# viswavi/speech-anonymization

Hardware: AMD Instinct MI355X
Metric: audio frames/sec (node), ConvAE+gender-adv train step (higher is better)
Workload: dtype bf16x3; 1 GPU; ConvAE recon0.1+sex0.9 adversarial train step (L1 recon + NLL), shape M: 32 utt/GPU x 161120 samples (T=1008 frames), Fbank x2 + norm + fwd + bwd + clip + Adam + Noam; batch_per_gpu=32, frames_per_utt=1008, parallelism=dp1

## Files before the change

include/sa_hip.h:

```cpp
#ifndef SA_HIP_H
#define SA_HIP_H
#ifdef __cplusplus
extern "C" {
#endif

#define SA_F32 0
#define SA_BF16 1
#define SA_BF16X3 2
#define SA_BF16X1F 3
#define SA_FP8 4
#define SA_F64 5
#define SA_MAX_TAPS 5
#define SA_COMM_ID_BYTES 128

typedef struct SaTaps {
  int ntaps[2];
  int off[2][SA_MAX_TAPS];
  int widx[2][SA_MAX_TAPS];
} SaTaps;

typedef struct SaConvArgs {
  const void* x;
  const void* wp;
  const float* bias;
// ... 27 lines not shown
int sa_conv_gemm_route(int dtype, int cin, int cout, int sa, int u, const SaConvArgs* a);

int sa_pack_weights(int dtype, const float* src, void* dst, int ntaps, int K, int N, int sk, int sn,
                    int st, void* stream);

typedef struct SaPackDesc {
  const float* src; void* dst;
  int dtype, ntaps, K, N, sk, sn, st, pad_;
  float* scale;
} SaPackDesc;
int sa_pack_weights_multi(const SaPackDesc* descs, int n, int blocks_per_image, void* stream);
int sa_pack_scales_multi(const SaPackDesc* descs, int n, void* stream);

typedef struct SaWgradArgs {
  const void* x;
  const void* dy;
  float* slabs;
  const float* s1; const float* t1; const float* s2; const float* t2; int swish;
  int B, Lin, Ldy, Mrows, chunk, nchunk;
  int ntaps; int off[SA_MAX_TAPS]; int ph[SA_MAX_TAPS];
  int x_pre;
  int dy_pre;
} SaWgradArgs;

int sa_wgrad(int dtype, int cin, int cout, int sa, int u, const SaWgradArgs* a, void* stream);
int sa_wgrad_kw(int cin, int cout);
int sa_wgrad_reduce(const float* slabs, float* dst, int nslab, int ntaps, int cin, int cout, int sk,
                    int sn, int st, int accumulate, void* stream);
#define SA_WRED_MAX 8
typedef struct SaWredDesc {
  const float* slabs; float* dst;
  int nslab, ntaps, cin, cout, sk, sn, st, accumulate, vec, pad_;
} SaWredDesc;
typedef struct SaWredMulti { int n, pad_; SaWredDesc d[SA_WRED_MAX]; } SaWredMulti;
int sa_wgrad_reduce_multi(const SaWredMulti* m, void* stream);

int sa_conv1toC(int dtype, const float* x, const float* w, const float* bias, void* y, int B, int L,
                int flip, float* stats, const void* ep_x, const float* ep_s1, const float* ep_t1,
                const float* ep_mean, const float* ep_rstd, void* stream);
int sa_conv1toC_ntiles(int L);
int sa_convCto1(int dtype, const void* x, const float* w, const float* bias, float* y, int B, int L,
                const float* s1, const float* t1, int swish, int flip, void* stream);
int sa_wgrad1C(int dtype, const float* u, const void* v, float* slabs, int B, int L, int chunk,
               int flip, const float* s1, const float* t1, int swish, void* stream);
int sa_wgrad1C_nchunk(int L, int chunk);
int sa_bwd1C(int dtype, const float* u, const void* v, const float* w, void* g, float* stats, float* slabs,
             int B, int L, int chunk, int flip, const float* s1, const float* t1, const float* mean,
             const float* rstd, void* stream);
int sa_sum_slabs(const float* slabs, float* dst, int nslab, int n, int accumulate, void* stream);

typedef struct SaEwArgs {
  const void* g; const void* g2; const void* x; void* out;
  const float* s1; const float* t1;
  const float* mean; const float* rstd;
  const float* c1; const float* c2; const float* c3;
  int actbwd, xp_is_act, relu_mask, bstride;
  float* stats;
  int B, L, ntiles;
} SaEwArgs;

int sa_ew_stats(int dtype, int C, const SaEwArgs* a, void* stream);
int sa_ew_apply(int dtype, int C, const SaEwArgs* a, void* stream);
int sa_ew_ntiles(int L);
int sa_sum_partials(const float* slabs, double* dst, int nbatch, int nslab, int n, void* stream);
int sa_sum_rows_d(const double* src, double* dst, int R, int n, void* stream);
int sa_fin_in_fwd(const double* sums, int B, int C, int n, const float* gamma, const float* beta,
                  float eps, float* mean, float* rstd, float* scale, float* shift, void* stream);
int sa_fin_bn_fwd(const double* sums, int R, int C, double count, const float* gamma, const float* beta,
                  float eps, float momentum, float* run_mean, float* run_var, float* mean,
                  float* rstd, float* scale, float* shift, const double* count_dev, void* stream);
int sa_fin_bn_eval(int C, const float* gamma, const float* beta, float eps, const float* run_mean,
                   const float* run_var, float* mean, float* rstd, float* scale, float* shift,
                   void* stream);
int sa_fin_norm_bwd(const double* sums, const double* lsums, int R, int groups, int C, double n,
                    const float* gamma, const float* mean, const float* rstd, float sign, float* c1,
                    float* c2, float* c3, float* dgamma, float* dbeta, const double* n_dev,
                    void* stream);
int sa_fin_bias(const double* sums, int B, int C, int ncomp, float* db, void* stream);

#define SA_FLATS_MAX 4
typedef struct SaFlat { float* p; long long n; } SaFlat;
typedef struct SaFlats { int n, pad_; SaFlat f[SA_FLATS_MAX]; } SaFlats;
int sa_clip_grads(const SaFlats* f, float max_norm, float eps, double* partials, float* total_norm, void* stream);
#define SA_BIAS_MAX 8
typedef struct SaBiasDesc {
  const float* part; double* rows; float* db;
  int nbatch, nslab, C, ncomp;
} SaBiasDesc;
typedef struct SaBiasMulti { int n, pad_; SaBiasDesc d[SA_BIAS_MAX]; } SaBiasMulti;
int sa_bias_multi(const SaBiasMulti* m, void* stream);

int sa_pool_fwd(int dtype, const void* r, const float* scale, const float* shift, float* part, int B,
                int L, int nseg, void* stream);
int sa_pool_nseg(int B);
int sa_pool_gather(const float* part, int B, int nseg, int L, double* sums, void* stream);
int sa_pool_fin(const double* sums, int B, int n, const float* noise, float eps, float* pooled,
                float* mean, float* stdraw, void* stream);
int sa_pool_gather_fin(const float* part, int B, int nseg, int L, const float* noise, int raw, float eps,
                       float* pooled, float* mean, float* stdraw, void* stream);
int sa_pool_bwd(int dtype, const void* r, const float* scale, const float* shift,
                const float* dpooled, const float* mean, const float* stdraw, void* g, int B, int L,
                const float* bn_mean, const float* bn_rstd, float* stats, void* stream);
int sa_dense(const float* X, int lda, const float* ps, const float* pt, const float* W, int sbk,
             int sbn, const float* bias, float* Y, int ldy, int M, int N, int K, int relu,
             void* stream);
int sa_colsums(const float* X, const float* H, const float* hmean, const float* hrstd, int M, int N,
               double* sums, float* out0, float* out1, void* stream);
int sa_bn2d_bwd(const float* G, const float* H, const double* sums, double count, const float* gamma,
                const float* mean, const float* rstd, int relu_mask, int M, int N, float* dH,
                const double* count_dev, void* stream);
int sa_dense_wgrad(const float* dY, const float* X, const float* ps, const float* pt, int M, int N,
                   int K, float* dW, void* stream);
int sa_log_softmax(const float* X, float* Y, int M, int N, void* stream);
int sa_log_softmax_bwd(const float* dY, const float* Y, float* dX, int M, int N, void* stream);
int sa_loss_workspace_bytes(void);
int sa_recon_loss(const float* a, const float* b, long long n, int kind, float* grad, float* loss,
                  void* workspace, void* stream);
int sa_cls_losses(const float* logp, const long long* label, int B, int NC, float* out, float* dnll,
                  float* dconf, void* stream);
int sa_cosine_loss(const float* x1, const float* x2, int B, int S, int D, float* rowloss,
                   float* loss, float* dx1, void* stream);
int sa_recon_loss_part(const float* a, const float* b, long long n, int kind, float* grad, float gscale,
                       void* workspace, void* stream);
int sa_step_loss(const void* workspace, long long n, const float* logp, const long long* label, int B, int NC,
                 float w_recon, float w_sex, float* out, float* dlogp, int* nonfinite, void* stream);

int sa_head_fwd(const float* pooled, const float* w1, const float* b1, const float* g1, const float* be1,
                float* rm1, float* rv1, const float* w2, const float* b2, const float* g2, const float* be2,
                float* rm2, float* rv2, const float* w3, const float* b3, float* h1, float* f1, float* h2,
                float* f2, float* logp, int M, float eps, float momentum, void* stream);
int sa_head_bwd(const float* dlogp, const float* logp, const float* pooled, const float* h1, const float* f1,
                const float* h2, const float* f2, const float* w1, const float* g1, const float* w2,
                const float* g2, const float* w3, float* dw1, float* db1, float* dg1, float* dbe1, float* dw2,
                float* db2, float* dg2, float* dbe2, float* dw3, float* db3, float* dpooled, int M, void* stream);
int sa_head_bwd_wide(const float* dlogp, const float* logp, const float* pooled, const float* h1, const float* f1,
                     const float* h2, const float* f2, const float* w1, const float* g1, const float* w2,
                     const float* g2, const float* w3, float* dw1, float* db1, float* dg1, float* dbe1, float* dw2,
                     float* db2, float* dg2, float* dbe2, float* dw3, float* db3, float* dpooled, int M,
                     void* stream);
int sa_head_max_rows(void);

int sa_tdnn_fwd(const float* x, const void* wp, const float* bias, const float* bn_s, const float* bn_t,
                float* y, int B, int T, int Cin, int Cout, int Npad, int K, int dil, float slope,
                unsigned char* mask, void* stream);
int sa_time_pool(const float* x, const float* lens, const float* noise, int B, int T, int C, float eps,
                 float* out, void* stream);
int sa_leaky_affine(const float* x, const float* s, const float* t, float slope, int M, int C, float* y,
                    void* stream);
int sa_tdnn_bwd_input(const float* dy, const unsigned char* mask, const float* bn_s, const void* wp,
                      float* dxe, int B, int T, int Cy, int Cred, int Cin, int Npad, int K, int dil,
                      float slope, void* stream);
int sa_tdnn_fold(const float* dxe, float* dx, int B, int T, int C, int pad, void* stream);
int sa_time_pool_bwd(const float* x, const float* lens, const float* g, const float* pooled, int B,
                     int T, int C, float eps, float* dx, void* stream);
int sa_leaky_affine_bwd(const float* dy, const float* x, const float* s, float slope, int M, int C,
                        float* dx, void* stream);

int sa_xv_tdnn_fwd_train(const float* x, const float* s_in, const float* t_in, const void* wp, const float* bias,
                         float* z, float* part, int B, int T, int Cin, int Cout, int Npad, int K, int dil,
                         float slope, void* stream);
int sa_xv_tdnn_ntiles(int T);
int sa_xv_colsums(const float* G, const float* H, const float* hmean, const float* hrstd, const float* c1,
                  const float* c2, const float* c3, float slope, float* out, int M, int N, int rows_per,
                  double* part, void* stream);
int sa_xv_tdnn_wgrad(const float* dpre, const float* x, const float* s_in, const float* t_in, float* part, int B,
                     int T, int Cin, int Cout, int K, int dil, int nsplit, int rows_per, void* stream);
// ... 176 lines not shown
```

speech-anonymization_amd/_lib.py:

```python
import ctypes as C
import os

import torch

_HERE = os.path.dirname(os.path.abspath(__file__))
LIB_PATH = os.environ.get("SA_HIP_LIB") or os.path.join(_HERE, "libsa_hip.so")

F32, BF16, BF16X3, BF16X1F, FP8, F64 = 0, 1, 2, 3, 4, 5
MAX_TAPS = 5

c_fp = C.POINTER(C.c_float)
vp = C.c_void_p


class SaTaps(C.Structure):
    _fields_ = [("ntaps", C.c_int * 2), ("off", (C.c_int * MAX_TAPS) * 2),
                ("widx", (C.c_int * MAX_TAPS) * 2)]


class SaConvArgs(C.Structure):
    _fields_ = [("x", vp), ("wp", vp), ("bias", vp), ("y", vp),
                ("s1", vp), ("t1", vp), ("s2", vp), ("t2", vp),
                ("swish", C.c_int), ("relu", C.c_int), ("stats", vp),
                ("B", C.c_int), ("Lin", C.c_int), ("Lout", C.c_int), ("ntiles", C.c_int),
                ("rowmin", C.c_int), ("nrows", C.c_int), ("wlo_off", C.c_int), ("taps", SaTaps),
                ("ep_mode", C.c_int), ("ep_xp_is_act", C.c_int), ("ep_bstride", C.c_int),
                ("ep_x", vp), ("ep_g2", vp), ("ep_s1", vp), ("ep_t1", vp), ("ep_mean", vp), ("ep_rstd", vp),
                ("a_out", vp),
                ("nb_x", vp), ("nb_c1", vp), ("nb_c2", vp), ("nb_c3", vp),
                ("nb_bstride", C.c_int), ("nb_relu_mask", C.c_int), ("nb_colsum", vp),
                ("ep_g2k1", vp), ("ep_g2k2", vp), ("ep_g2k3", vp), ("pro_stats", vp), ("wscale", vp),
                ("tile_rows", C.c_int), ("pad2_", C.c_int)]


class SaPackDesc(C.Structure):
    _fields_ = [("src", vp), ("dst", vp), ("dtype", C.c_int), ("ntaps", C.c_int), ("K", C.c_int),
                ("N", C.c_int), ("sk", C.c_int), ("sn", C.c_int), ("st", C.c_int), ("pad_", C.c_int),
                ("scale", vp)]


class SaWgradArgs(C.Structure):
    _fields_ = [("x", vp), ("dy", vp), ("slabs", vp),
                ("s1", vp), ("t1", vp), ("s2", vp), ("t2", vp), ("swish", C.c_int),
                ("B", C.c_int), ("Lin", C.c_int), ("Ldy", C.c_int), ("Mrows", C.c_int),
                ("chunk", C.c_int), ("nchunk", C.c_int),
                ("ntaps", C.c_int), ("off", C.c_int * MAX_TAPS), ("ph", C.c_int * MAX_TAPS),
                ("x_pre", C.c_int), ("dy_pre", C.c_int)]


class SaEwArgs(C.Structure):
    _fields_ = [("g", vp), ("g2", vp), ("x", vp), ("out", vp),
                ("s1", vp), ("t1", vp), ("mean", vp), ("rstd", vp),
                ("c1", vp), ("c2", vp), ("c3", vp),
                ("actbwd", C.c_int), ("xp_is_act", C.c_int), ("relu_mask", C.c_int),
                ("bstride", C.c_int), ("stats", vp),
                ("B", C.c_int), ("L", C.c_int), ("ntiles", C.c_int)]


BIAS_MAX = 8


class SaBiasDesc(C.Structure):
    _fields_ = [("part", vp), ("rows", vp), ("db", vp),
                ("nbatch", C.c_int), ("nslab", C.c_int), ("C", C.c_int), ("ncomp", C.c_int)]


class SaBiasMulti(C.Structure):
    _fields_ = [("n", C.c_int), ("pad_", C.c_int), ("d", SaBiasDesc * BIAS_MAX)]


WRED_MAX = 8
FLATS_MAX = 4


class SaFlat(C.Structure):
    _fields_ = [("p", vp), ("n", C.c_longlong)]


class SaFlats(C.Structure):
    _fields_ = [("n", C.c_int), ("pad_", C.c_int), ("f", SaFlat * FLATS_MAX)]



class SaWredDesc(C.Structure):
    _fields_ = [("slabs", vp), ("dst", vp)] + [(k, C.c_int) for k in ("nslab", "ntaps", "cin", "cout", "sk", "sn", "st",
                                                                      "accumulate", "vec", "pad_")]


class SaWredMulti(C.Structure):
    _fields_ = [("n", C.c_int), ("pad_", C.c_int), ("d", SaWredDesc * WRED_MAX)]


SYMBOLS = [
    "sa_conv_gemm", "sa_abi_sizeof", "sa_conv_gemm_ntiles", "sa_conv_gemm_ntiles_tm", "sa_conv_gemm_set_tile_rows",
    "sa_conv_gemm_set_impl", "sa_conv_gemm_route", "sa_pack_weights", "sa_pack_weights_multi", "sa_pack_scales_multi", "sa_wgrad", "sa_wgrad_kw", "sa_wgrad_reduce",
    "sa_conv1toC", "sa_conv1toC_ntiles", "sa_convCto1", "sa_wgrad1C", "sa_wgrad1C_nchunk", "sa_bwd1C",
    "sa_sum_slabs", "sa_ew_stats", "sa_ew_apply", "sa_ew_ntiles",
    "sa_sum_partials", "sa_sum_rows_d", "sa_fin_in_fwd", "sa_fin_bn_fwd", "sa_fin_bn_eval", "sa_fin_norm_bwd", "sa_fin_bias",
    "sa_pool_fwd", "sa_pool_nseg", "sa_pool_gather", "sa_pool_fin", "sa_pool_gather_fin", "sa_pool_bwd", "sa_dense", "sa_colsums",
    "sa_bn2d_bwd", "sa_dense_wgrad", "sa_log_softmax", "sa_log_softmax_bwd",
    "sa_loss_workspace_bytes", "sa_recon_loss", "sa_cls_losses", "sa_cosine_loss", "sa_recon_loss_part", "sa_step_loss",
    "sa_tdnn_fwd", "sa_time_pool", "sa_leaky_affine", "sa_tdnn_bwd_input", "sa_tdnn_fold", "sa_time_pool_bwd",
    "sa_leaky_affine_bwd", "sa_cluster_mi", "sa_fbank", "sa_fbank_table_elems", "sa_fbank_ntiles", "sa_fbank_scratch_bytes", "sa_fbank_normalize", "sa_fbank_normalize_pair",
    "sa_comm_unique_id", "sa_comm_init", "sa_comm_world", "sa_comm_allreduce", "sa_comm_allreduce_inline", "sa_comm_join", "sa_comm_ncalls",
    "sa_comm_destroy", "sa_head_fwd", "sa_head_bwd", "sa_head_bwd_wide", "sa_head_max_rows",
    "sa_add_layernorm_fwd", "sa_layernorm_bwd", "sa_reflect_pad_fwd", "sa_reflect_pad_bwd", "sa_ln_leaky_fwd", "sa_ln_leaky_bwd", "sa_bias_multi", "sa_asr_block0_fwd", "sa_asr_block0_bwd", "sa_wgrad_reduce_multi", "sa_clip_grads",
    "sa_xv_tdnn_fwd_train", "sa_xv_tdnn_ntiles", "sa_xv_colsums", "sa_xv_tdnn_wgrad", "sa_xv_wgrad_reduce",
    "sa_xv_tdnn_dgrad", "sa_xv_pool_affine", "sa_xv_pool_affine_bwd",
    "sa_fc_tiles", "sa_fc_groups", "sa_fc_nparam", "sa_fc_nhead", "sa_fc_max_rows", "sa_fc_enc_fwd", "sa_fc_bn_fin",
    "sa_fc_mid_fwd", "sa_fc_head_fwd", "sa_fc_head_bwd", "sa_fc_mid_bwd", "sa_fc_bn_bwd_fin", "sa_fc_enc_bwd",
    "sa_fc_wreduce", "sa_fc_recon_fwd",
    "sa_wav_augment_tile", "sa_wav_augment_max_chunks", "sa_wav_abs_sums", "sa_noise_scales", "sa_wav_augment",
    "sa_specaug_warp_sums", "sa_specaug_finalize", "sa_specaug_fill",
    "sa_gl_tile", "sa_mel_to_mag", "sa_gl_istft", "sa_gl_project",
    "sa_yin_dim", "sa_yin_f0", "sa_pitch_ratio", "sa_pitch_stretch_mag", "sa_pitch_resample",
    "sa_env_dim", "sa_env_warp",
    "sa_mcadams_dim", "sa_mcadams",
    "sa_stoi_dim", "sa_stoi",
    "sa_pv_dim", "sa_pv_synth",
    "sa_contour_dim", "sa_pitch_contour", "sa_pv_synth_map", "sa_env_warp_frames", "sa_pitch_resample_map",
    "sa_f0v_dim", "sa_f0_candidates", "sa_f0_viterbi",
    "sa_f0cmp_dim", "sa_f0_compare",
    "sa_mcd_dim", "sa_mcd",
    "sa_psola_dim", "sa_psola_marks", "sa_psola_plan", "sa_psola_ola",
    "sa_formant_dim", "sa_formant_tracks", "sa_formant_compare",
    "sa_pole_warp_dim", "sa_pole_warp", "sa_formant_centre",
]

_lib = None


class SaHipError(RuntimeError):
    pass


def load():
    global _lib
    if _lib is None:
        if not os.path.exists(LIB_PATH):
            raise SaHipError(
                f"{LIB_PATH} not found: build it with `python -c 'import __graft_entry__ as g; "
                "g.build()'` (hipcc --offload-arch=gfx950). There is no CPU fallback.")
        _lib = C.CDLL(LIB_PATH)
        for s in SYMBOLS:
            getattr(_lib, s).restype = C.c_int
        _lib.sa_pv_workspace_bytes.restype = C.c_longlong
        _lib.sa_psola_workspace_bytes.restype = C.c_longlong
        for i, rec in enumerate((SaConvArgs, SaWgradArgs, SaEwArgs, SaPackDesc, SaTaps, SaBiasMulti, SaWredMulti, SaFlats)):
            if _lib.sa_abi_sizeof(i) != C.sizeof(rec):
                raise SaHipError(f"{rec.__name__}: binding has {C.sizeof(rec)} bytes, {LIB_PATH} "
                                 f"{_lib.sa_abi_sizeof(i)} -- rebuild the library (stale build?)")
    return _lib


def stream():
    return C.c_void_p(torch._C._cuda_getCurrentRawStream(torch._C._cuda_getDevice()))


def ptr(t):
    if t is None:
        return None
    assert t.is_cuda and t.is_contiguous(), "HIP kernels take contiguous device tensors"
    return C.c_void_p(t.data_ptr())


def check(rc, what):
    if rc != 0:
        raise SaHipError(f"{what} failed with code {rc}")


def dt_code(dtype):
    if dtype == torch.float32:
        return F32
    if dtype == torch.bfloat16:
        return BF16
    raise SaHipError(f"unsupported activation dtype {dtype}")


_taps_cache = {}


def make_taps(phases):
    key = tuple(tuple(p) for p in phases)
    t = _taps_cache.get(key)
    if t is not None:
        return t
    t = _taps_cache[key] = SaTaps()
    for ph, lst in enumerate(phases):
        t.ntaps[ph] = len(lst)
        for i, (off, wi) in enumerate(lst):
            t.off[ph][i] = off
            t.widx[ph][i] = wi
    return t
```

speech-anonymization_amd/brain.py:

```python
import enum
import os
import types

import torch

from . import distributed as sdist


class Stage(enum.Enum):
    TRAIN = 1
    VALID = 2
    TEST = 3


class EpochCounter:

    def __init__(self, limit):
        self.current, self.limit = 0, int(limit)

    def __iter__(self):
        return self

    def __next__(self):
        if self.current < self.limit:
            self.current += 1
            return self.current
        raise StopIteration


class NoamScheduler:

    def __init__(self, lr_initial, n_warmup_steps, model_size=None):
        self.lr_initial, self.n_warmup_steps = lr_initial, n_warmup_steps
        self.current_lr, self.n_steps = lr_initial, 0
        self.normalize = n_warmup_steps ** 0.5 if model_size is None else model_size ** (-0.5)

    def __call__(self, opt):
        self.n_steps += 1
        current_lr = getattr(opt, "_sa_host_lr", None)
        if current_lr is None:
            current_lr = opt.param_groups[0]["lr"]
        lr = self.lr_initial * self.normalize * min(self.n_steps ** (-0.5),
                                                    self.n_steps * self.n_warmup_steps ** (-1.5))
        for g in opt.param_groups:
            if torch.is_tensor(g["lr"]):
                g["lr"].fill_(lr)
            else:
                g["lr"] = lr
        opt._sa_host_lr = lr
        self.current_lr = current_lr
        return current_lr, lr

    def state_dict(self):
        return {"losses": [], "n_steps": self.n_steps}

    def load_state_dict(self, sd):
        self.n_steps = sd["n_steps"]


class Batch:

    def __init__(self, wavs, lens, gender, tokens_bos=None, ids=None):
        self.sig = (wavs, lens)
        self.gender = gender
        self.tokens_bos = (tokens_bos if tokens_bos is not None
                           else torch.ones(wavs.shape[0], 1, dtype=torch.long), lens)
        self.id = ids

    def to(self, device):
        w, l = self.sig
        tb, tl = self.tokens_bos
        out = Batch.__new__(Batch)
        out.sig = (w.to(device, non_blocking=True), l.to(device, non_blocking=True))
        out.gender = self.gender.to(device, non_blocking=True)
        out.tokens_bos = (tb.to(device, non_blocking=True), tl.to(device, non_blocking=True))
        out.id = self.id
        return out


def settle_python_heap():
    import gc
    gc.collect()
    gc.freeze()


class Brain:
    GC_FREEZE_STEP = 8

    def __init__(self, modules=None, opt_class=None, hparams=None, run_opts=None, checkpointer=None):
        run_opts = dict(run_opts or {})
        self.device = torch.device(run_opts.get("device", "cuda:0" if torch.cuda.is_available() else "cpu"))
        if self.device.type == "cuda":
            torch.cuda.set_device(self.device)
        self.max_grad_norm = float(run_opts.get("max_grad_norm", 5.0))
        self.nonfinite_patience = int(run_opts.get("nonfinite_patience", 3))
        self.lazy_finite_check = bool(run_opts.get("lazy_finite_check", True))
        self.hip_graph = bool(run_opts.get("hip_graph", False)) and self.device.type == "cuda"
        self.gc_freeze = bool(run_opts.get("gc_freeze", True))
        self.fused_clip = bool(run_opts.get("fused_clip", os.environ.get("SA_FUSED_CLIP", "1") == "1"))
        self.front_end_once = bool(run_opts.get("front_end_once", os.environ.get("SA_FRONT_END_ONCE", "1") == "1"))
        self.step_tail = bool(run_opts.get("step_tail", os.environ.get("SA_STEP_TAIL", "1") == "1"))
        self.distributed_launch = bool(run_opts.get("distributed_launch", sdist.is_distributed()))
        self.modules = torch.nn.ModuleDict(modules or {})
        self.dp_batch_sizes = run_opts.get("dp_batch_sizes", "equal")
        self.opt_class = opt_class
        self.hparams = types.SimpleNamespace(**(hparams or {}))
        self.checkpointer = checkpointer
        self.step, self.nonfinite_count, self.optimizer = 0, 0, None
        self.avg_train_loss = 0.0

    def compute_forward(self, batch, stage):
        raise NotImplementedError

    def compute_objectives(self, predictions, batch, stage):
        raise NotImplementedError

    def on_stage_start(self, stage, epoch=None):
        pass

    def on_stage_end(self, stage, stage_loss, epoch=None):
        pass

    def on_fit_start(self):
        self.modules.to(self.device)
        for m in self.modules.values():
            if hasattr(m, "dp_batch_sizes"):
                m.dp_batch_sizes = self.dp_batch_sizes
        self.init_optimizers()
        if self.checkpointer is not None:
            if self.optimizer is not None:
                self.checkpointer.add_recoverable("optimizer", self.optimizer)
            self.resumed_from = self.checkpointer.recover_if_possible(device=self.device, brain=self)

    def init_optimizers(self):
        if self.opt_class is not None and self.optimizer is None:
            params = list(self.modules.parameters())
            base = getattr(self.opt_class, "func", self.opt_class)
            given = getattr(self.opt_class, "keywords", None) or {}
            if base is torch.optim.Adam and "fused" not in given and params and all(p.is_cuda for p in params):
                try:
                    if self.hip_graph:
                        self.optimizer = self.opt_class(params, fused=True, capturable=True)
                        for g in self.optimizer.param_groups:
                            self.optimizer._sa_host_lr = float(g["lr"])
                            g["lr"] = torch.tensor(float(g["lr"]), dtype=torch.float32, device=self.device)
                    else:
                        self.optimizer = self.opt_class(params, fused=True)
                    return
                except (TypeError, RuntimeError):
                    self.hip_graph = False
            self.optimizer = self.opt_class(params)

    def check_gradients(self, loss):
        bad = self._count_nonfinite(loss)
        if bad:
            self.nonfinite_count += bad
            if self.nonfinite_count > self.nonfinite_patience:
                raise ValueError("Loss is not finite and patience is exhausted.")
            if not (self.lazy_finite_check and loss.is_cuda):
                return False
        params = getattr(self, "_clip_params", None)
        if params is None:
            params = self._clip_params = list(self.modules.parameters())
        flats = self._grad_flats(params) if self.fused_clip else None
        if flats:
            from . import ops
            ops.clip_flats(flats, self.max_grad_norm)
        else:
            torch.nn.utils.clip_grad_norm_(params, self.max_grad_norm)
        return True

    def _grad_flats(self, params):
        model = self.modules["ConvAE"] if "ConvAE" in self.modules else None
        flats = getattr(model, "_last_flats", None) if model is not None else None
        if not flats:
            return None
        spans = [(f.data_ptr(), f.data_ptr() + 4 * f.numel(), f.numel()) for f in flats]
        seen = [0] * len(flats)
        for p in params:
            g = p.grad
            if g is None:
                continue
            if g.dtype != torch.float32 or not g.is_contiguous():
                return None
            a = g.data_ptr()
            for i, (lo, hi, _) in enumerate(spans):
                if lo <= a < hi:
                    seen[i] += g.numel()
                    break
            else:
                return None
        if any(n != span[2] for n, span in zip(seen, spans)):
            return None
        return flats

    def _count_nonfinite(self, loss):
        if not (self.lazy_finite_check and loss.is_cuda):
            return 0 if bool(torch.isfinite(loss)) else 1
        st = self._finite_counter(loss.device)
        new = self._poll_nonfinite()
        if st.pop("counted", None) is not loss:
            st["dev"].add_((~torch.isfinite(loss.detach())).to(torch.int32))
        st["host"].copy_(st["dev"], non_blocking=True)
        if not torch.cuda.is_current_stream_capturing():
            st["event"].record()
            st["pending"] = True
        return new

    def _finite_counter(self, device):
        st = getattr(self, "_finite_state", None)
        if st is None:
            st = self._finite_state = dict(dev=torch.zeros((), dtype=torch.int32, device=device),
                                           host=torch.zeros((), dtype=torch.int32).pin_memory(),
                                           event=torch.cuda.Event(), seen=0, pending=False)
        return st

    def _poll_nonfinite(self, wait=False):
        st = getattr(self, "_finite_state", None)
        if st is None or not st["pending"]:
            return 0
        if wait:
            st["event"].synchronize()
        elif not st["event"].query():
            return 0
        st["pending"] = False
        total = int(st["host"])
        new, st["seen"] = total - st["seen"], total
        return max(new, 0)

    def fit_batch(self, batch):
        outputs = self.compute_forward(batch, Stage.TRAIN)
        loss = self.compute_objectives(outputs, batch, Stage.TRAIN)
        loss.backward()
        if self.check_gradients(loss):
            self.optimizer.step()
        self.optimizer.zero_grad()
        return loss.detach()

    def evaluate_batch(self, batch, stage):
        out = self.compute_forward(batch, stage=stage)
        return self.compute_objectives(out, batch, stage=stage).detach()

    def update_average(self, loss, avg_loss):
        if not loss.is_cuda:
            if torch.isfinite(loss):
                avg_loss -= avg_loss / self.step
                avg_loss += float(loss) / self.step
            return avg_loss
        if not torch.is_tensor(avg_loss):
            avg_loss = torch.full((), float(avg_loss), device=loss.device, dtype=torch.float32)
        new = avg_loss + (loss.detach().float() - avg_loss) / self.step
        return torch.where(torch.isfinite(loss), new, avg_loss)

    def fit(self, epoch_counter, train_set, valid_set=None, progressbar=False, **_):
        self.on_fit_start()
        for epoch in epoch_counter:
            self.on_stage_start(Stage.TRAIN, epoch)
            self.modules.train()
            self.nonfinite_count = 0
            self.avg_train_loss = 0.0
            self.step = 0
            for batch in train_set:
                self.step += 1
                loss = self.fit_batch(batch)
                self.avg_train_loss = self.update_average(loss, self.avg_train_loss)
                if self.gc_freeze and self.step == self.GC_FREEZE_STEP and not self.__dict__.get("_gc_frozen"):
                    settle_python_heap()
                    self._gc_frozen = True
            self.nonfinite_count += self._poll_nonfinite(wait=True)
            if self.nonfinite_count > self.nonfinite_patience:
                raise ValueError("Loss is not finite and patience is exhausted.")
            self.avg_train_loss = float(self.avg_train_loss)
            self.on_stage_end(Stage.TRAIN, self.avg_train_loss, epoch)
            if valid_set is not None:
                self.on_stage_start(Stage.VALID, epoch)
                self.modules.eval()
                avg, n = 0.0, 0
                with torch.no_grad():
                    for batch in valid_set:
                        n += 1
                        avg += (float(self.evaluate_batch(batch, Stage.VALID)) - avg) / n
                self.on_stage_end(Stage.VALID, avg, epoch)

    def on_evaluate_start(self, max_key=None, min_key=None):
        pass

    def evaluate(self, test_set, max_key=None, min_key=None, **_):
        self.on_evaluate_start(max_key=max_key, min_key=min_key)
        self.on_stage_start(Stage.TEST, None)
        self.modules.eval()
        avg, n = 0.0, 0
        with torch.no_grad():
            for batch in test_set:
                n += 1
                avg += (float(self.evaluate_batch(batch, Stage.TEST)) - avg) / n
        self.on_stage_end(Stage.TEST, avg, None)
        return avg


class SexAnonymizationTraining(Brain):

    @staticmethod
    def _sig_key(wavs, wav_lens):
        return tuple((t.data_ptr(), tuple(t.shape), t.dtype, t._version) for t in (wavs, wav_lens))

    def features(self, wavs, wav_lens):
        stash, self._target_stash = self.__dict__.get("_target_stash"), None
        if stash is not None and stash[0] == self._sig_key(wavs, wav_lens):
            return stash[1]
        feats = self.hparams.compute_features(wavs)
        current_epoch = self.hparams.epoch_counter.current
        pad = 36 if self.hparams.model_type != "fcae" else None
        return self.modules.normalize(feats, wav_lens, epoch=current_epoch, pad_multiple=pad)

    def _features_pair(self, wavs, wav_lens):
        feats = self.hparams.compute_features(wavs)
        pad = 36 if self.hparams.model_type != "fcae" else None
        inp, target = self.modules.normalize.forward_pair(feats, wav_lens, epoch=self.hparams.epoch_counter.current,
# ... 86 lines not shown
                and isinstance(hp.loss_sex_classification, losses.NLLLoss)):
            return False
        w = (hp.recon_loss_weight, hp.sex_loss_weight, hp.utility_loss_weight)
        if not all(isinstance(x, (int, float)) and x == x and abs(x) != float("inf") for x in w):
            return False
        if not (w[2] == 0 or (w[2] > 0 and getattr(self, "asr_brain", None) is None)):
            return False
        if predictions is not None:
            recon, logp = predictions
            return bool(recon.is_cuda and recon.requires_grad and logp.requires_grad and logp.dim() == 2
                        and recon.dtype == logp.dtype == torch.float32)
        return True

    def _objectives_native(self, recon, logp, feats, label):
        from . import ops
        hp = self.hparams
        B = recon.shape[0]
        st = self._finite_counter(recon.device) if self.lazy_finite_check else None
        label = torch.as_tensor(label, device=logp.device).long().contiguous()
        out, d_recon, d_logp = ops.step_loss(
            recon.detach().view(B, -1).contiguous(), feats.detach().view(B, -1).contiguous().float(),
            hp.loss_reconstruction.kind, logp.detach().contiguous(), label,
            float(hp.recon_loss_weight), float(hp.sex_loss_weight), nonfinite=st["dev"] if st else None)
        loss = out[2]
        self.last_losses = dict(recon=out[0], sex=out[1])
        self._tail = (loss, (recon, logp), (d_recon.view_as(recon), d_logp))
        if st is not None:
            st["counted"] = loss
        return loss

    def _backward(self, loss, accumulate=False):
        tail, self._tail = self.__dict__.get("_tail"), None
        if tail is not None and tail[0] is loss:
            torch.autograd.backward(tail[1], tail[2])
        elif accumulate:
            (loss / self.hparams.gradient_accumulation).backward()
        else:
            loss.backward()

    def apply_epoch_schedule(self):
        hp = self.hparams
        if not getattr(hp, "epoch_parity_schedule", False):
            return
        joint = hp.epoch_counter.current % 2 == 0
        if joint:
            hp.recon_loss_weight, hp.sex_loss_weight = 0.0, 0.8
            hp.utility_loss_weight, hp.confusion_loss_weight = 0.2, 0.0
        else:
            hp.recon_loss_weight, hp.sex_loss_weight, hp.utility_loss_weight = 0.0, 0.5, 0.0
        for name, param in self.modules.ConvAE.named_parameters():
            param.requires_grad = ("sex_classifier" not in name) if joint else ("sex_classifier" in name)

    def _zero_grads_of_frozen(self):
        st = self.optimizer.state
        for group in self.optimizer.param_groups:
            for p in group["params"]:
                if p.grad is None and not p.requires_grad and p in st and len(st[p]):
                    z = getattr(self, "_zero_grad_cache", None)
                    if z is None:
                        z = self._zero_grad_cache = {}
                    g = z.get(p)
                    if g is None:
                        g = z[p] = torch.zeros_like(p)
                    p.grad = g

    GRAPH_WARMUP = 3

    def _graph_key(self, batch):
        hp = self.hparams
        wavs, lens = batch.sig
        nrm = self.modules["normalize"] if "normalize" in self.modules else None
        upd = nrm is not None and hp.epoch_counter.current < getattr(nrm, "update_until_epoch", 0)
        st = self.optimizer.state if self.optimizer is not None else {}
        params = list(self.modules.ConvAE.parameters())
        tok = batch.tokens_bos[0]
        return (tuple(wavs.shape), str(wavs.dtype), hp.model_type, float(hp.recon_loss_weight),
                float(hp.sex_loss_weight), float(hp.utility_loss_weight),
                float(getattr(hp, "confusion_loss_weight", 0.0)), bool(upd),
                tuple(p.requires_grad for p in params),
                tuple(bool(st.get(p)) for p in params if not p.requires_grad),
                tuple(tok.shape), getattr(self, "asr_brain", None) is not None,
                self.front_end_once, bool(not upd and getattr(nrm, "_count_positive", False)),
                self.__dict__.get("_specaug") is not None,
                self._native_tail())

    def _step_core(self, batch):
        predictions = self.compute_forward(batch, Stage.TRAIN)
        loss = self.compute_objectives(predictions, batch, Stage.TRAIN)
        self._backward(loss)
        if getattr(self.hparams, "epoch_parity_schedule", False):
            self._zero_grads_of_frozen()
        self.check_gradients(loss)
        self.optimizer.step()
        return loss.detach()

    def _fit_batch_graph(self, batch):
        batch = batch.to(self.device)
        key = self._graph_key(batch)
        graphs = self.__dict__.setdefault("_graphs", {})
        ent = graphs.get(key)
        if ent is None:
            ent = graphs[key] = {"seen": 0}
        if "graph" not in ent:
            ent["seen"] += 1
            if ent["seen"] <= self.GRAPH_WARMUP:
                self.optimizer.zero_grad(set_to_none=True)
                loss = self._step_core(batch)
                self.optimizer.zero_grad()
                self.hparams.noam_annealing(self.optimizer)
                return loss
            wavs, lens = batch.sig
            ent["wav"], ent["lens"] = wavs.clone(), lens.clone()
            ent["gender"] = batch.gender.clone()
            tok, tok_lens = batch.tokens_bos
            ent["tok"], ent["tok_lens"] = tok.clone(), tok_lens.clone()
            ent["batch"] = Batch(ent["wav"], ent["lens"], ent["gender"], tokens_bos=ent["tok"], ids=batch.id)
            ent["batch"].tokens_bos = (ent["tok"], ent["tok_lens"])
            torch.cuda.synchronize()
            self.nonfinite_count += self._poll_nonfinite(wait=True)
            g = torch.cuda.CUDAGraph()
            self.optimizer.zero_grad(set_to_none=True)
            aug = self.__dict__.get("_specaug")
            if aug is not None:
                ent["specaug"] = self._specaug_shapes[tuple(wavs.shape)]
                aug.draw(*ent["specaug"], device=self.device)
                self._specaug_drawn = True
            try:
                with torch.cuda.graph(g):
                    ent["loss"] = self._step_core(ent["batch"])
            finally:
                self._specaug_drawn = False
            ent["graph"] = g
        elif "specaug" in ent:
            self._specaug.draw(*ent["specaug"], device=self.device)
        wavs, lens = batch.sig
        ent["wav"].copy_(wavs, non_blocking=True)
        ent["lens"].copy_(lens, non_blocking=True)
        ent["gender"].copy_(batch.gender, non_blocking=True)
        ent["tok"].copy_(batch.tokens_bos[0], non_blocking=True)
        ent["tok_lens"].copy_(batch.tokens_bos[1], non_blocking=True)
        ent["batch"].id = batch.id
        bad = self._poll_nonfinite()
        if bad:
            self.nonfinite_count += bad
            if self.nonfinite_count > self.nonfinite_patience:
                raise ValueError("Loss is not finite and patience is exhausted.")
        ent["graph"].replay()
        st = getattr(self, "_finite_state", None)
        if st is not None:
            st["event"].record()
            st["pending"] = True
        self.hparams.noam_annealing(self.optimizer)
        return ent["loss"]

    def fit_batch(self, batch):
        self._target_stash, self._in_fit_batch, self._tail = None, True, None
        try:
            return self._fit_batch(batch)
        finally:
            self._target_stash, self._in_fit_batch, self._tail = None, False, None

    def _fit_batch(self, batch):
        self.apply_epoch_schedule()
        if (self.hip_graph and self.hparams.gradient_accumulation == 1 and sdist.capturable()
                and self.optimizer is not None):
            return self._fit_batch_graph(batch)
        if self.front_end_once:
            batch = batch.to(self.device)
        predictions = self.compute_forward(batch, Stage.TRAIN)
        loss = self.compute_objectives(predictions, batch, Stage.TRAIN)
        self._backward(loss, accumulate=True)
        if self.step % self.hparams.gradient_accumulation == 0:
            if getattr(self.hparams, "epoch_parity_schedule", False):
                self._zero_grads_of_frozen()
            self.check_gradients(loss)
            self.optimizer.step()
            self.optimizer.zero_grad()
            self.hparams.noam_annealing(self.optimizer)
        return loss.detach()

    def evaluate_batch(self, batch, stage):
        with torch.no_grad():
            predictions = self.compute_forward(batch, stage=stage)
            loss = self.compute_objectives(predictions, batch, stage=stage)
        return loss.detach()

    def load_external_classifier(self):
        ext = getattr(self.hparams, "external_classifier", None)
        if ext is not None:
            ext.eval()
            ext.to(self.device)
        return ext

    def on_stage_start(self, stage, epoch=None):
        from .metrics import AccuracyStats, SimilarityMetricsStats
        self.external_classifier = self.load_external_classifier()
        if stage == Stage.TRAIN:
            self._specaug = self.spec_augment()
            if self._specaug is not None:
                self.__dict__.setdefault("_specaug_shapes", {})
                self._specaug.reseed(epoch, sdist.rank())
        if stage != Stage.TRAIN:
            self.sex_classification_acc = AccuracyStats()
            self.sex_classification_acc_extern = AccuracyStats()
            self.sex_classification_acc_extern_orig = AccuracyStats()
            self.utility_similarity_aggregator = SimilarityMetricsStats()

    def on_evaluate_start(self, max_key=None, min_key=None):
        if self.checkpointer is None:
            return
        ckpts = self.checkpointer.find_checkpoints(max_key=max_key, min_key=min_key)
        if not ckpts:
            return
        sd = self.checkpointer.average_checkpoints(ckpts, recoverable_name="model", device=self.device)
        model = getattr(self.hparams, "model", None)
        if model is not None:
            model.load_state_dict(sd, strict=False)
            model.eval()

    def on_stage_end(self, stage, stage_loss, epoch=None):
        stats = {"loss": stage_loss}
        if stage == Stage.TRAIN:
            self.train_stats = stats
            return
        stats["ACC"] = self.sex_classification_acc.summarize()
        if self.external_classifier is not None:
            stats["ACC_external"] = self.sex_classification_acc_extern.summarize()
            stats["ACC_external_orig"] = self.sex_classification_acc_extern_orig.summarize()
        if self.utility_similarity_aggregator.denom:
            stats["Utility_Retention"] = float(self.utility_similarity_aggregator.summarize())
        self.valid_stats = stats
        logger = getattr(self.hparams, "train_logger", None)
        if stage == Stage.VALID and sdist.if_main_process() and logger is not None:
            na = self.hparams.noam_annealing
            logger.log_stats(stats_meta={"epoch": epoch, "lr": na.current_lr, "steps": na.n_steps,
                                         "optimizer": self.optimizer.__class__.__name__},
                             train_stats=self.train_stats, valid_stats=stats)
        if stage == Stage.VALID and sdist.if_main_process() and self.checkpointer is not None:
            keys = {k: stats[k] for k in ("ACC_external", "Utility_Retention") if k in stats}
            self.checkpointer.save_and_keep_only(self, epoch, dict(stats, **keys),
                                                 max_keys=[k for k in ("Utility_Retention",) if k in stats],
                                                 min_keys=[k for k in ("ACC_external",) if k in stats],
                                                 num_to_keep=5)


class FileTrainLogger:

    def __init__(self, save_file):
        self.save_file = save_file

    @staticmethod
    def _fmt(d):
        out = []
        for k, v in d.items():
            if isinstance(v, float) and 1.0 < v < 100.0:
                v = f"{v:.2f}"
            elif isinstance(v, float):
                v = f"{v:.2e}"
            out.append(f"{k}: {v}")
# ... 11 lines not shown
```

speech-anonymization_amd/ops.py:

```python
import collections
import ctypes as C
import functools
import sys

import torch

from . import _lib as L

UP2 = [[(1, 0), (0, 2), (-1, 4)], [(1, 1), (0, 3)]]


def taps_conv(K, dil, pad):
    return [[(k * dil - pad, k) for k in range(K)]]


def taps_conv_dgrad_s1(K, dil, pad):
    return [[(pad - k * dil, k) for k in range(K)]]


def taps_convT_dgrad(K=5, pad=2):
    return [[(k - pad, k) for k in range(K)]]


CONVT_WG_TAPS = [(1, 0), (1, 1), (0, 0), (0, 1), (-1, 0)]
# ... 658 lines not shown
    rows = x.numel() // d
    y = torch.empty_like(x)
    s = torch.empty_like(x) if save else None
    stat = torch.empty(rows, 2, dtype=torch.float32, device=x.device) if save else None
    L.check(L.load().sa_add_layernorm_fwd(_f(x), _f(r), _f(gamma), _f(beta), _f(y), _f(s), _f(stat), rows, d,
                                          C.c_float(eps), L.stream()), "sa_add_layernorm_fwd")
    return y, s, stat


def layernorm_bwd(dy, s, stat, gamma):
    d = s.shape[-1]
    ds = torch.empty_like(s)
    L.check(L.load().sa_layernorm_bwd(_f(dy), _f(s), _f(stat), _f(gamma), _f(ds), s.numel() // d, d, L.stream()),
            "sa_layernorm_bwd")
    return ds


def reflect_pad(x):
    B, T, F_, Cc = x.shape
    y = torch.empty(B, T + 2, F_ + 2, Cc, dtype=x.dtype, device=x.device)
    L.check(L.load().sa_reflect_pad_fwd(_f(x), _f(y), B, T, F_, Cc, L.stream()), "sa_reflect_pad_fwd")
    return y


def reflect_pad_bwd(dy):
    B, T2, F2, Cc = dy.shape
    dx = torch.empty(B, T2 - 2, F2 - 2, Cc, dtype=dy.dtype, device=dy.device)
    L.check(L.load().sa_reflect_pad_bwd(_f(dy), _f(dx), B, T2 - 2, F2 - 2, Cc, L.stream()), "sa_reflect_pad_bwd")
    return dx


def ln_leaky(x, gamma, beta, eps, slope, save):
    d = gamma.numel()
    rows = x.numel() // d
    y = torch.empty_like(x)
    stat = torch.empty(rows, 2, dtype=torch.float32, device=x.device) if save else None
    L.check(L.load().sa_ln_leaky_fwd(_f(x), _f(gamma), _f(beta), _f(y), _f(stat), rows, d, C.c_float(eps),
                                     C.c_float(slope), L.stream()), "sa_ln_leaky_fwd")
    return y, stat


def ln_leaky_bwd(dy, x, stat, gamma, beta, slope):
    d = gamma.numel()
    dx = torch.empty_like(x)
    L.check(L.load().sa_ln_leaky_bwd(_f(dy), _f(x), _f(stat), _f(gamma), _f(beta), _f(dx), x.numel() // d, d,
                                     C.c_float(slope), L.stream()), "sa_ln_leaky_bwd")
    return dx


def asr_block0(x, w, bias, gamma, beta, eps, slope, save):
    B, T, F_ = x.shape
    Cc = w.shape[0]
    To = (T - 1) // 2 + 1
    y = torch.empty(B, To, (F_ - 1) // 2 + 1, Cc, dtype=x.dtype, device=x.device)
    stat = torch.empty(B * To, 2, dtype=torch.float32, device=x.device) if save else None
    L.check(L.load().sa_asr_block0_fwd(_f(x), _f(w), _f(bias), _f(gamma), _f(beta), _f(y), _f(stat), B, T, F_, Cc,
                                       C.c_float(eps), C.c_float(slope), L.stream()), "sa_asr_block0_fwd")
    return y, stat


def asr_block0_bwd(dy, x, w, bias, gamma, beta, stat, slope):
    B, T, F_ = x.shape
    To = (T - 1) // 2 + 1
    part = torch.empty(B * To, 3, F_ + 2, dtype=torch.float32, device=x.device)
    dx = torch.empty_like(x)
    L.check(L.load().sa_asr_block0_bwd(_f(dy), _f(x), _f(w), _f(bias), _f(gamma), _f(beta), _f(stat), _f(part), _f(dx),
                                       B, T, F_, w.shape[0], C.c_float(slope), L.stream()), "sa_asr_block0_bwd")
    return dx


def clip_flats(flats, max_norm, eps=1e-6):
    f = L.SaFlats()
    f.n = len(flats)
    for d, t in zip(f.f, flats):
        d.p, d.n = t.data_ptr(), t.numel()
    dev = flats[0].device
    partials = torch.empty(L.FLATS_MAX * 64, dtype=torch.float64, device=dev)
    total = torch.empty((), dtype=torch.float32, device=dev)
    L.check(L.load().sa_clip_grads(C.byref(f), C.c_float(max_norm), C.c_float(eps), _f(partials), _f(total), L.stream()),
            "sa_clip_grads")
    return total


def _aug_in(t, what, dtype=torch.float32, shape=None, family="augmentation"):
    if not torch.is_tensor(t) or not t.is_cuda:
        raise L.SaHipError(f"{what}: the {family} kernels take GPU tensors (no CPU fallback)")
    if t.dtype != dtype:
        raise L.SaHipError(f"{what}: expected {dtype}, got {t.dtype}")
    if not t.is_contiguous():
        raise L.SaHipError(f"{what}: expected a contiguous tensor")
    if shape is not None and tuple(t.shape) != tuple(shape):
        raise L.SaHipError(f"{what}: expected shape {tuple(shape)}, got {tuple(t.shape)}")
    return t


def wav_abs_sums(wav, noise=None):
    if _aug_in(wav, "wav").dim() != 2 or wav.numel() == 0:
        raise L.SaHipError(f"wav: expected [B, L] with B, L >= 1, got {tuple(wav.shape)}")
    B, Lw = wav.shape
    if noise is not None:
        _aug_in(noise, "noise", shape=(B, Lw))
    sums = torch.empty(2, B, dtype=torch.float64, device=wav.device)
    L.check(L.load().sa_wav_abs_sums(_f(wav), _f(noise), B, Lw, _f(sums), L.stream()), "sa_wav_abs_sums")
    return sums


def noise_scales(sums, lens, snr, Lw):
    B = _aug_in(lens, "lens").numel()
    _aug_in(sums, "sums", torch.float64, (2, B))
    _aug_in(snr, "snr", shape=(B,))
    scales = torch.empty(B, 2, dtype=torch.float32, device=sums.device)
    L.check(L.load().sa_noise_scales(_f(sums), _f(lens), _f(snr), B, int(Lw), _f(scales), L.stream()),
            "sa_noise_scales")
    return scales


def wav_augment(wav, noise, scales, plan_words, R, Lp, S_in, S_out, W, first_min, first_max):
    if _aug_in(wav, "wav").dim() != 2 or wav.numel() == 0:
        raise L.SaHipError(f"wav: expected [B, L] with B, L >= 1, got {tuple(wav.shape)}")
    B, Lw = wav.shape
    if R not in (B, 2 * B):
        raise L.SaHipError(f"R = {R}: the output has B = {B} rows, or 2 B with noise rows")
    if R == 2 * B:
        _aug_in(noise, "noise", shape=(B, Lw))
        _aug_in(scales, "scales", shape=(B, 2))
    else:
        noise = scales = None
    from . import augment
    need = S_out + S_out * W + 101 + R * (1 + 2 * augment.max_chunks())
    if _aug_in(plan_words, "plan", torch.int32).numel() < need:
        raise L.SaHipError(f"plan: {plan_words.numel()} words, the geometry needs {need}")
    out = torch.empty(R, Lp, dtype=torch.float32, device=wav.device)
    L.check(L.load().sa_wav_augment(_f(wav), _f(noise), _f(scales), _f(plan_words), B, Lw, R, int(Lp), int(S_in),
                                    int(S_out), int(W), int(first_min), int(first_max), _f(out), L.stream()),
            "sa_wav_augment")
    return out


SPECAUG_TILE = 32


def _specaug_shape(x, what):
    if _aug_in(x, what).dim() != 3:
        raise L.SaHipError(f"{what}: expected [B, T, F], got {tuple(x.shape)}")
    B, T, F = x.shape
    if B < 1 or B > 65535 or T < 1 or F < 4 or F % 4 or F > 128:
        raise L.SaHipError(f"{what}: [B, T, F] = {tuple(x.shape)} -- B in 1..65535, T >= 1, F a multiple of 4 up to 128")
    if x.data_ptr() % 16:
        raise L.SaHipError(f"{what}: expected 16-byte aligned storage")
    return B, T, F


def _specaug_plan(words, B, T):
    from . import specaug
    need = specaug.plan_words(B, T)
    if _aug_in(words, "plan", torch.int32).numel() < need:
        raise L.SaHipError(f"plan: {words.numel()} words, the geometry needs {need}")


def specaug_warp_sums(x, plan_words):
    B, T, F = _specaug_shape(x, "x")
    _specaug_plan(plan_words, B, T)
    out = torch.empty_like(x)
    part = torch.empty(-(-T // SPECAUG_TILE) * B, 2, dtype=torch.float64, device=x.device)
    L.check(L.load().sa_specaug_warp_sums(_f(x), _f(plan_words), B, T, F, _f(out), _f(part), L.stream()),
            "sa_specaug_warp_sums")
# ... 668 lines not shown
```

Baseline: 3.936 million frames/s.

## Replace torch fused Adam with native multi-tensor HIP Adam kernel

Adds a custom HIP Adam kernel driven by a cached device-side table of per-tensor records and a block→(tensor,chunk) map, so all parameters update in one launch and gradients are read straight from the flat gradient buffers. It runs in place of torch's fused Adam when the optimizer is plain Adam, falling back otherwise, and the graph cache key gains the new flag. It also disables Python GC during graph capture. The cost targeted is optimizer-step launch and dispatch overhead. The price is extra table and state management and bitwise-matching arithmetic done in double precision.

```diff
diff --git a/include/sa_hip.h b/include/sa_hip.h
--- a/include/sa_hip.h
+++ b/include/sa_hip.h
@@ -133,6 +133,15 @@
 typedef struct SaFlat { float* p; long long n; } SaFlat;
 typedef struct SaFlats { int n, pad_; SaFlat f[SA_FLATS_MAX]; } SaFlats;
 int sa_clip_grads(const SaFlats* f, float max_norm, float eps, double* partials, float* total_norm, void* stream);
+#define SA_ADAM_CHUNK 1024
+typedef struct SaAdamRec {
+  float* p; float* m; float* v; const float* step; const float* g;
+  long long goff, n;
+  int gbase, pad_;
+} SaAdamRec;
+int sa_adam_record_bytes(void);
+int sa_adam_step(const SaAdamRec* table, int ntensors, const int* map, int nblocks, const SaFlats* bases,
+                 const float* lr_dev, double lr, double beta1, double beta2, double eps, void* stream);
 #define SA_BIAS_MAX 8
 typedef struct SaBiasDesc {
   const float* part; double* rows; float* db;
diff --git a/speech-anonymization_amd/_lib.py b/speech-anonymization_amd/_lib.py
--- a/speech-anonymization_amd/_lib.py
+++ b/speech-anonymization_amd/_lib.py
@@ -80,6 +80,14 @@
 class SaFlats(C.Structure):
     _fields_ = [("n", C.c_int), ("pad_", C.c_int), ("f", SaFlat * FLATS_MAX)]
 
+
+
+class SaAdamRec(C.Structure):
+    _fields_ = [("p", vp), ("m", vp), ("v", vp), ("step", vp), ("g", vp),
+                ("goff", C.c_longlong), ("n", C.c_longlong), ("gbase", C.c_int), ("pad_", C.c_int)]
+
+
+ADAM_CHUNK = 1024
 
 
 class SaWredDesc(C.Structure):
@@ -105,6 +113,7 @@
     "sa_comm_unique_id", "sa_comm_init", "sa_comm_world", "sa_comm_allreduce", "sa_comm_allreduce_inline", "sa_comm_join", "sa_comm_ncalls",
     "sa_comm_destroy", "sa_head_fwd", "sa_head_bwd", "sa_head_bwd_wide", "sa_head_max_rows",
     "sa_add_layernorm_fwd", "sa_layernorm_bwd", "sa_reflect_pad_fwd", "sa_reflect_pad_bwd", "sa_ln_leaky_fwd", "sa_ln_leaky_bwd", "sa_bias_multi", "sa_asr_block0_fwd", "sa_asr_block0_bwd", "sa_wgrad_reduce_multi", "sa_clip_grads",
+    "sa_adam_record_bytes", "sa_adam_step",
     "sa_xv_tdnn_fwd_train", "sa_xv_tdnn_ntiles", "sa_xv_colsums", "sa_xv_tdnn_wgrad", "sa_xv_wgrad_reduce",
     "sa_xv_tdnn_dgrad", "sa_xv_pool_affine", "sa_xv_pool_affine_bwd",
     "sa_fc_tiles", "sa_fc_groups", "sa_fc_nparam", "sa_fc_nhead", "sa_fc_max_rows", "sa_fc_enc_fwd", "sa_fc_bn_fin",
@@ -150,6 +159,9 @@
             if _lib.sa_abi_sizeof(i) != C.sizeof(rec):
                 raise SaHipError(f"{rec.__name__}: binding has {C.sizeof(rec)} bytes, {LIB_PATH} "
                                  f"{_lib.sa_abi_sizeof(i)} -- rebuild the library (stale build?)")
+        if _lib.sa_adam_record_bytes() != C.sizeof(SaAdamRec):
+            raise SaHipError(f"SaAdamRec: binding has {C.sizeof(SaAdamRec)} bytes, {LIB_PATH} "
+                             f"{_lib.sa_adam_record_bytes()} -- rebuild the library (stale build?)")
     return _lib
 
 
diff --git a/speech-anonymization_amd/brain.py b/speech-anonymization_amd/brain.py
--- a/speech-anonymization_amd/brain.py
+++ b/speech-anonymization_amd/brain.py
@@ -100,6 +100,7 @@
         self.fused_clip = bool(run_opts.get("fused_clip", os.environ.get("SA_FUSED_CLIP", "1") == "1"))
         self.front_end_once = bool(run_opts.get("front_end_once", os.environ.get("SA_FRONT_END_ONCE", "1") == "1"))
         self.step_tail = bool(run_opts.get("step_tail", os.environ.get("SA_STEP_TAIL", "1") == "1"))
+        self.native_adam = bool(run_opts.get("native_adam", os.environ.get("SA_NATIVE_ADAM", "1") == "1"))
         self.distributed_launch = bool(run_opts.get("distributed_launch", sdist.is_distributed()))
         self.modules = torch.nn.ModuleDict(modules or {})
         self.dp_batch_sizes = run_opts.get("dp_batch_sizes", "equal")
@@ -150,6 +151,14 @@
                 except (TypeError, RuntimeError):
                     self.hip_graph = False
             self.optimizer = self.opt_class(params)
+
+    def optimizer_step(self):
+        if self.native_adam and self.device.type == "cuda":
+            from . import ops
+            model = self.modules["ConvAE"] if "ConvAE" in self.modules else None
+            if ops.adam_step(self.optimizer, getattr(model, "_last_flats", None)):
+                return
+        self.optimizer.step()
 
     def check_gradients(self, loss):
         bad = self._count_nonfinite(loss)
@@ -233,7 +242,7 @@
         loss = self.compute_objectives(outputs, batch, Stage.TRAIN)
         loss.backward()
         if self.check_gradients(loss):
-            self.optimizer.step()
+            self.optimizer_step()
         self.optimizer.zero_grad()
         return loss.detach()
 
@@ -486,7 +495,7 @@
                 tuple(tok.shape), getattr(self, "asr_brain", None) is not None,
                 self.front_end_once, bool(not upd and getattr(nrm, "_count_positive", False)),
                 self.__dict__.get("_specaug") is not None,
-                self._native_tail())
+                self._native_tail(), self.native_adam)
 
     def _step_core(self, batch):
         predictions = self.compute_forward(batch, Stage.TRAIN)
@@ -495,7 +504,7 @@
         if getattr(self.hparams, "epoch_parity_schedule", False):
             self._zero_grads_of_frozen()
         self.check_gradients(loss)
-        self.optimizer.step()
+        self.optimizer_step()
         return loss.detach()
 
     def _fit_batch_graph(self, batch):
@@ -529,10 +538,16 @@
                 ent["specaug"] = self._specaug_shapes[tuple(wavs.shape)]
                 aug.draw(*ent["specaug"], device=self.device)
                 self._specaug_drawn = True
+            import gc
+            gc.collect()
+            gc_was_on = gc.isenabled()
+            gc.disable()
             try:
                 with torch.cuda.graph(g):
                     ent["loss"] = self._step_core(ent["batch"])
             finally:
+                if gc_was_on:
+                    gc.enable()
                 self._specaug_drawn = False
             ent["graph"] = g
         elif "specaug" in ent:
@@ -578,7 +593,7 @@
             if getattr(self.hparams, "epoch_parity_schedule", False):
                 self._zero_grads_of_frozen()
             self.check_gradients(loss)
-            self.optimizer.step()
+            self.optimizer_step()
             self.optimizer.zero_grad()
             self.hparams.noam_annealing(self.optimizer)
         return loss.detach()
diff --git a/speech-anonymization_amd/csrc/sa_optim.hip b/speech-anonymization_amd/csrc/sa_optim.hip
--- /dev/null
+++ b/speech-anonymization_amd/csrc/sa_optim.hip
@@ -0,0 +1,69 @@
+#include "sa_common.h"
+
+struct SaAdamCoef { double b1, b2, omb1, omb2, eps; float step_size, bc2s; };
+
+__device__ static inline void sa_adam_math(const SaAdamCoef& k, float g, float& p, float& m, float& v) {
+#pragma clang fp contract(off)
+  const double gd = (double)g;
+  m = (float)fma(k.b1, (double)m, k.omb1 * gd);
+  v = (float)fma(k.b2, (double)v, (k.omb2 * gd) * gd);
+  const float denom = (float)((double)(sqrtf(v) / k.bc2s) + k.eps);
+  p = p - (k.step_size * m) / denom;
+}
+
+__global__ __launch_bounds__(256) void sa_adam_kernel(const SaAdamRec* __restrict__ table, int ntensors,
+                                                      const int* __restrict__ map, SaFlats bases,
+                                                      const float* __restrict__ lr_dev, double lr, double beta1,
+                                                      double beta2, double eps) {
+#pragma clang fp contract(off)
+  const int t = map[2 * blockIdx.x], chunk = map[2 * blockIdx.x + 1];
+  if (t < 0 || t >= ntensors || chunk < 0) return;
+  const SaAdamRec r = table[t];
+  const long long i0 = (long long)chunk * SA_ADAM_CHUNK + 4 * (long long)threadIdx.x;
+  if (i0 >= r.n || r.gbase >= bases.n) return;
+  const float* gp = r.gbase >= 0 ? bases.f[r.gbase].p + r.goff : r.g;
+  const double step = (double)*r.step;
+  const double lrd = lr_dev ? (double)*lr_dev : lr;
+  SaAdamCoef k;
+  k.b1 = beta1; k.b2 = beta2; k.eps = eps;
+  k.omb1 = 1.0 - beta1; k.omb2 = 1.0 - beta2;
+  const float bc1 = (float)(1.0 - pow(beta1, step));
+  k.bc2s = (float)sqrt(1.0 - pow(beta2, step));
+  k.step_size = (float)(lrd / (double)bc1);
+  float* pp = r.p + i0; float* mp = r.m + i0; float* vp = r.v + i0; gp += i0;
+  const bool vec = i0 + 4 <= r.n &&
+                   ((((uintptr_t)pp) | ((uintptr_t)mp) | ((uintptr_t)vp) | ((uintptr_t)gp)) & 15) == 0;
+  if (vec) {
+    float4 p4 = *reinterpret_cast<const float4*>(pp), m4 = *reinterpret_cast<const float4*>(mp);
+    float4 v4 = *reinterpret_cast<const float4*>(vp);
+    const float4 g4 = *reinterpret_cast<const float4*>(gp);
+    sa_adam_math(k, g4.x, p4.x, m4.x, v4.x);
+    sa_adam_math(k, g4.y, p4.y, m4.y, v4.y);
+    sa_adam_math(k, g4.z, p4.z, m4.z, v4.z);
+    sa_adam_math(k, g4.w, p4.w, m4.w, v4.w);
+    *reinterpret_cast<float4*>(pp) = p4;
+    *reinterpret_cast<float4*>(mp) = m4;
+    *reinterpret_cast<float4*>(vp) = v4;
+  } else {
+    const int cnt = r.n - i0 < 4 ? (int)(r.n - i0) : 4;
+    for (int j = 0; j < cnt; ++j) {
+      float p = pp[j], m = mp[j], v = vp[j];
+      sa_adam_math(k, gp[j], p, m, v);
+      pp[j] = p; mp[j] = m; vp[j] = v;
+    }
+  }
+}
+
+extern "C" int sa_adam_record_bytes(void) { return (int)sizeof(SaAdamRec); }
+
+extern "C" int sa_adam_step(const SaAdamRec* table, int ntensors, const int* map, int nblocks, const SaFlats* bases,
+                            const float* lr_dev, double lr, double beta1, double beta2, double eps, void* stream) {
+  if (!table || !map || !bases || ntensors <= 0 || nblocks <= 0 || bases->n < 0 || bases->n > SA_FLATS_MAX) return -22;
+  for (int j = 0; j < bases->n; ++j)
+    if (!bases->f[j].p) return -22;
+  hipStream_t st = reinterpret_cast<hipStream_t>(stream);
+  hipLaunchKernelGGL(sa_adam_kernel, dim3(nblocks), dim3(256), 0, st, table, ntensors, map, *bases, lr_dev, lr, beta1,
+                     beta2, eps);
+  hipError_t e = hipGetLastError();
+  return e == hipSuccess ? 0 : -(int)e;
+}
diff --git a/speech-anonymization_amd/ops.py b/speech-anonymization_amd/ops.py
--- a/speech-anonymization_amd/ops.py
+++ b/speech-anonymization_amd/ops.py
@@ -764,6 +764,114 @@
     return total
 
 
+def _adam_plain(opt):
+    from torch.optim import optimizer as _o
+    if type(opt) is not torch.optim.Adam:
+        return False
+    if getattr(opt, "grad_scale", None) is not None or getattr(opt, "found_inf", None) is not None:
+        return False
+    if (opt._optimizer_step_pre_hooks or opt._optimizer_step_post_hooks or _o._global_optimizer_pre_hooks
+            or _o._global_optimizer_post_hooks):
+        return False
+    for g in opt.param_groups:
+        if (not g.get("fused") or g["weight_decay"] != 0 or g["amsgrad"] or g["maximize"] or g.get("differentiable")
+                or g.get("decoupled_weight_decay")):
+            return False
+        if any(torch.is_tensor(b) for b in g["betas"]) or torch.is_tensor(g["eps"]):
+            return False
+        lr = g["lr"]
+        if torch.is_tensor(lr) and not (lr.is_cuda and lr.dtype == torch.float32 and lr.numel() == 1):
+            return False
+    return True
+
+
+def _adam_group(opt, group, spans):
+    st, key, steps, dev = opt.state, [], [], None
+    f32 = torch.float32
+    for p in group["params"]:
+        g = p.grad
+        if g is None:
+            continue
+        s = st.get(p)
+        if not s:
+            return None
+        step, m, v = s["step"], s["exp_avg"], s["exp_avg_sq"]
+        n = p.numel()
+        if dev is None:
+            dev = p.device
+            if dev.type != "cuda":
+                return None
+        for t in (p, g, m, v):
+            if (t.dtype is not f32 or t.device != dev or t.layout is not torch.strided or t.numel() != n
+                    or not t.is_contiguous()):
+                return None
+        if step.dtype is not f32 or step.device != dev or step.numel() != 1 or n == 0:
+            return None
+        a = g.data_ptr()
+        rec = (p.data_ptr(), m.data_ptr(), v.data_ptr(), step.data_ptr(), n, -1, a)
+        for i, (lo, hi) in enumerate(spans):
+            if lo <= a and a + 4 * n <= hi:
+                rec = rec[:5] + (i, (a - lo) // 4)
+                break
+        key.append(rec)
+        steps.append(step)
+    return tuple(key), steps, dev
+
+
+def _adam_table(key, dev):
+    arr = (L.SaAdamRec * len(key))()
+    blocks = []
+    for t, (r, (p, m, v, step, n, gbase, goff)) in enumerate(zip(arr, key)):
+        r.p, r.m, r.v, r.step, r.n, r.gbase = p, m, v, step, n, gbase
+        r.g, r.goff = (goff, 0) if gbase < 0 else (None, goff)
+        blocks.extend((t, c) for c in range(-(-n // L.ADAM_CHUNK)))
+    table = torch.frombuffer(bytearray(bytes(arr)), dtype=torch.uint8).to(dev)
+    bmap = torch.tensor(blocks, dtype=torch.int32).to(dev)
+    return table, bmap, len(key), len(blocks)
+
+
+def adam_step(opt, flats=None):
+    if not _adam_plain(opt):
+        return False
+    flats = list(flats or ())[:L.FLATS_MAX]
+    spans = [(f.data_ptr(), f.data_ptr() + 4 * f.numel()) for f in flats]
+    cache = opt.__dict__.setdefault("_sa_adam_tables", {})
+    captured = opt.__dict__.setdefault("_sa_adam_captured", [])
+    capturing = torch.cuda.is_current_stream_capturing()
+    plans = []
+    for gi, group in enumerate(opt.param_groups):
+        plan = _adam_group(opt, group, spans)
+        if plan is None:
+            return False
+        key, steps, dev = plan
+        if not key:
+            continue
+        ent = cache.get(gi)
+        if ent is None or ent[0] != key:
+            ent = next((e for e in captured if e[0] == key), None)
+            if ent is None:
+                if capturing:
+                    return False
+                ent = (key,) + _adam_table(key, dev)
+            cache[gi] = ent
+        plans.append((group, steps, ent))
+    if capturing:
+        captured.extend(ent for _, _, ent in plans if not any(ent is e for e in captured))
+    bases = L.SaFlats()
+    bases.n = len(flats)
+    for d, (lo, hi) in zip(bases.f, spans):
+        d.p, d.n = lo, (hi - lo) // 4
+    lib = L.load()
+    for group, steps, (_, table, bmap, nt, nblocks) in plans:
+        torch._foreach_add_(steps, 1)
+        lr = group["lr"]
+        lr_dev, lr_host = (_f(lr), 0.0) if torch.is_tensor(lr) else (None, float(lr))
+        b1, b2 = group["betas"]
+        L.check(lib.sa_adam_step(_f(table), nt, _f(bmap), nblocks, C.byref(bases), lr_dev, C.c_double(lr_host),
+                                 C.c_double(b1), C.c_double(b2), C.c_double(group["eps"]), L.stream()), "sa_adam_step")
+    return True
+
+
 def _aug_in(t, what, dtype=torch.float32, shape=None, family="augmentation"):
     if not torch.is_tensor(t) or not t.is_cuda:
         raise L.SaHipError(f"{what}: the {family} kernels take GPU tensors (no CPU fallback)")
```

Result: faster. 3.976 million frames/s (median of 6 runs) (+1.0%).
